# wesselb/gpar

Hardware: AMD Instinct MI355X
Metric: logpdf_per_s (higher is better)
Workload: dtype f64; 1 GPU; C3 dense GPAR log marginal likelihood: n=16384 m=4 p=8 markov=2 linear+nonlinear output kernels, noise=0.1, inputs resident in HBM

## Files before the change

### gpar_amd/csrc/gemm_f64.h

```cpp
#pragma once
#include "common.h"
#include <stdlib.h>

namespace gpar {

constexpr int GEMM_BM = 128;
constexpr int GEMM_BN = 128;
constexpr int GEMM_BK = 16;
constexpr int GEMM_LDKC = 18;
constexpr int GEMM_LDMC = 144;
constexpr int GEMM_TILE = 2304;
constexpr int GEMM_LDS_BYTES = 4 * GEMM_TILE * 8;
#ifndef GPAR_GEMM_EPI_PRIO
#define GPAR_GEMM_EPI_PRIO 3
#endif
#ifndef GPAR_GEMM_NT_STORE
#define GPAR_GEMM_NT_STORE 1
#endif
#ifndef GPAR_GEMM_PRELOAD_C
#define GPAR_GEMM_PRELOAD_C 1
#endif
constexpr int GEMM_LDT = 66;

struct GemmArgs {
    const double* A;
    const double* B;
    double* C;
    int m, n, k;
    int lda, ldb, ldc;
    double alpha, beta;
    int flags;
    int tiles_m, tiles_n;
    int fastA, fastB, fastC;
    int ksplit;
    long long part_stride;
    long long batch_a, batch_b, batch_c;
    int nfull, ntail;
    long long* stamps;
    long long* stage_stamps;
    const int* pred;
    int pred_sense;
};

typedef double gpar_d2 __attribute__((ext_vector_type(2)));
typedef double gpar_d4 __attribute__((ext_vector_type(4)));

template <bool KC, int FAST, int ROWS = 128>
__device__ __forceinline__ void gemm_gload(const double* __restrict__ g, int ld, int r0, int rmax, int k0,
                                           int kmax, bool lower, int t, gpar_d2 (&reg)[ROWS / 32]) {
    if (FAST) {
#pragma unroll
        for (int q = 0; q < ROWS / 32; ++q) {
            const int c = t + 256 * q;
            if (KC) {
                const int r = c >> 3, kk = (c & 7) * 2;
                const int row = (FAST == 2) ? min(r0 + r, rmax - 1) : r0 + r;
                reg[q] = *reinterpret_cast<const gpar_d2*>(g + (size_t)row * ld + k0 + kk);
            } else {
                const int kk = c / (ROWS / 2), r = (c % (ROWS / 2)) * 2;
                reg[q] = *reinterpret_cast<const gpar_d2*>(g + (size_t)(k0 + kk) * ld + r0 + r);
            }
        }
    } else {
#pragma unroll
        for (int q = 0; q < ROWS / 32; ++q) {
            const int c = t + 256 * q;
            int r, kk, r1, kk1;
            if (KC) { r = r0 + (c >> 3); kk = k0 + (c & 7) * 2; r1 = r; kk1 = kk + 1; }
            else { kk = k0 + c / (ROWS / 2); r = r0 + (c % (ROWS / 2)) * 2; r1 = r + 1; kk1 = kk; }
            const bool ok0 = r < rmax && kk < kmax && (!lower || kk <= r);
            const bool ok1 = r1 < rmax && kk1 < kmax && (!lower || kk1 <= r1);
            const int rc = min(r, rmax - 1), kc = min(kk, kmax - 1), rc1 = min(r1, rmax - 1), kc1 = min(kk1, kmax - 1);
            const double v0 = KC ? g[(size_t)rc * ld + kc] : g[(size_t)kc * ld + rc];
            const double v1 = KC ? g[(size_t)rc1 * ld + kc1] : g[(size_t)kc1 * ld + rc1];
            reg[q] = gpar_d2{ok0 ? v0 : 0.0, ok1 ? v1 : 0.0};
        }
    }
}

template <bool KC, int ROWS = 128>
__device__ __forceinline__ void gemm_sstore(double* __restrict__ s, int t, const gpar_d2 (&reg)[ROWS / 32]) {
#pragma unroll
    for (int q = 0; q < ROWS / 32; ++q) {
        const int c = t + 256 * q;
        if (KC) {
            const int r = c >> 3, kk = (c & 7) * 2;
            *reinterpret_cast<gpar_d2*>(s + r * GEMM_LDKC + kk) = reg[q];
        } else {
            const int kk = c / (ROWS / 2), r = (c % (ROWS / 2)) * 2;
            *reinterpret_cast<gpar_d2*>(s + kk * GEMM_LDMC + r) = reg[q];
        }
    }
}

template <bool A_KC, bool B_KC, int FAST, int BM>
__device__ __forceinline__ void gemm_mainloop(const GemmArgs& p, double* smem, gpar_d4 (&acc)[BM / 32][4], int m0, int n0,
                                              int kbeg, int kend, int nk, bool a_lower, int t, int lane, int wm, int wn) {
    gpar_d2 ra[BM / 32], rb[4];
    if (nk > 0) {
        gemm_gload<A_KC, FAST, BM>(p.A, p.lda, m0, p.m, kbeg, kend, a_lower, t, ra);
        gemm_gload<B_KC, FAST>(p.B, p.ldb, n0, p.n, kbeg, kend, false, t, rb);
        gemm_sstore<A_KC, BM>(smem, t, ra);
        gemm_sstore<B_KC>(smem + GEMM_TILE, t, rb);
    }
    __syncthreads();

    const int l15 = lane & 15, lk = lane >> 4;
    for (int kt = 0; kt < nk; ++kt) {
        const double* As = smem + (kt & 1) * 2 * GEMM_TILE;
        const double* Bs = As + GEMM_TILE;
        const bool more = kt + 1 < nk;
        __builtin_amdgcn_s_setprio(1);
#pragma unroll
        for (int k4 = 0; k4 < 4; ++k4) {
            const int kk = k4 * 4 + lk;
            double af[BM / 32], bf[4];
#pragma unroll
            for (int mi = 0; mi < BM / 32; ++mi) {
                const int r = wm * (BM / 2) + 16 * mi + l15;
                af[mi] = A_KC ? As[r * GEMM_LDKC + kk] : As[kk * GEMM_LDMC + r];
            }
#pragma unroll
            for (int nj = 0; nj < 4; ++nj) {
                const int c = wn * 64 + 16 * nj + l15;
                bf[nj] = B_KC ? Bs[c * GEMM_LDKC + kk] : Bs[kk * GEMM_LDMC + c];
            }
#pragma unroll
            for (int mi = 0; mi < BM / 32; ++mi)
#pragma unroll
                for (int nj = 0; nj < 4; ++nj)
                    acc[mi][nj] = __builtin_amdgcn_mfma_f64_16x16x4f64(af[mi], bf[nj], acc[mi][nj], 0, 0, 0);
            if (k4 == 0 && more) {
                gemm_gload<A_KC, FAST, BM>(p.A, p.lda, m0, p.m, kbeg + (kt + 1) * GEMM_BK, kend, a_lower, t, ra);
                gemm_gload<B_KC, FAST>(p.B, p.ldb, n0, p.n, kbeg + (kt + 1) * GEMM_BK, kend, false, t, rb);
            }
        }
        __builtin_amdgcn_s_setprio(0);
        if (more) {
            double* An = smem + ((kt + 1) & 1) * 2 * GEMM_TILE;
            gemm_sstore<A_KC, BM>(An, t, ra);
            gemm_sstore<B_KC>(An + GEMM_TILE, t, rb);
        }
        __syncthreads();
    }
}

template <bool A_KC, bool B_KC, int FAST, int BM>
__device__ __forceinline__ void gemm_stage(const GemmArgs& p, const double* __restrict__ As, const double* __restrict__ Bs,
                                           gpar_d4 (&acc)[BM / 32][4], int m0, int n0, int knext, int kend, int t, int l15, int lk,
                                           int wm, int wn, gpar_d2 (&ra)[BM / 32], gpar_d2 (&rb)[4]) {
    __builtin_amdgcn_s_setprio(1);
#pragma unroll
    for (int k4 = 0; k4 < 4; ++k4) {
        const int kk = k4 * 4 + lk;
        double af[BM / 32], bf[4];
#pragma unroll
        for (int mi = 0; mi < BM / 32; ++mi) {
            const int r = wm * (BM / 2) + 16 * mi + l15;
            af[mi] = A_KC ? As[r * GEMM_LDKC + kk] : As[kk * GEMM_LDMC + r];
        }
#pragma unroll
        for (int nj = 0; nj < 4; ++nj) {
            const int c = wn * 64 + 16 * nj + l15;
            bf[nj] = B_KC ? Bs[c * GEMM_LDKC + kk] : Bs[kk * GEMM_LDMC + c];
        }
#pragma unroll
        for (int mi = 0; mi < BM / 32; ++mi)
#pragma unroll
            for (int nj = 0; nj < 4; ++nj) {
                acc[mi][nj] = __builtin_amdgcn_mfma_f64_16x16x4f64(af[mi], bf[nj], acc[mi][nj], 0, 0, 0);
            }
        if (k4 == 0) {
            gemm_gload<A_KC, FAST, BM>(p.A, p.lda, m0, p.m, knext, kend, false, t, ra);
            gemm_gload<B_KC, FAST>(p.B, p.ldb, n0, p.n, knext, kend, false, t, rb);
        }
    }
    __builtin_amdgcn_s_setprio(0);
}

template <bool A_KC, bool B_KC, int FAST, int BM, bool PRELOAD = false>
__device__ __forceinline__ void gemm_mainloop_pf2(const GemmArgs& p, double* smem, gpar_d4 (&acc)[BM / 32][4], int m0, int n0,
                                                  int kbeg, int kend, int nk, int t, int lane, int wm, int wn) {
    static_assert(FAST != 0, "branch-free loads only");
    if (nk <= 0) return;
    gpar_d2 ra0[BM / 32], rb0[4], ra1[BM / 32], rb1[4];
    double* buf0 = smem;
    double* buf1 = smem + 2 * GEMM_TILE;
    const int klast = kbeg + (nk - 1) * GEMM_BK;
    gemm_gload<A_KC, FAST, BM>(p.A, p.lda, m0, p.m, kbeg, kend, false, t, ra0);
    gemm_gload<B_KC, FAST>(p.B, p.ldb, n0, p.n, kbeg, kend, false, t, rb0);
    gemm_gload<A_KC, FAST, BM>(p.A, p.lda, m0, p.m, min(kbeg + GEMM_BK, klast), kend, false, t, ra1);
    gemm_gload<B_KC, FAST>(p.B, p.ldb, n0, p.n, min(kbeg + GEMM_BK, klast), kend, false, t, rb1);
    if (PRELOAD) {
        const int wmu = __builtin_amdgcn_readfirstlane(wm), wnu = __builtin_amdgcn_readfirstlane(wn);
        const double* cw = p.C + (size_t)(m0 + wmu * (BM / 2)) * p.ldc + n0 + wnu * 64;
        const unsigned voff = ((unsigned)(lane >> 4) * (unsigned)p.ldc + (unsigned)(lane & 15)) * 8u;
        const double sgn = p.alpha;
#pragma unroll
        for (int mi = 0; mi < BM / 32; ++mi)
#pragma unroll
            for (int v = 0; v < 4; ++v) {
                const char* cr = reinterpret_cast<const char*>(cw + (size_t)(16 * mi + 4 * v) * p.ldc);
#pragma unroll
                for (int nj = 0; nj < 4; ++nj) acc[mi][nj][v] = sgn * *reinterpret_cast<const double*>(cr + voff + 128 * nj);
            }
    }
    gemm_sstore<A_KC, BM>(buf0, t, ra0);
    gemm_sstore<B_KC>(buf0 + GEMM_TILE, t, rb0);
    __syncthreads();
    const int l15 = lane & 15, lk = lane >> 4;
#ifdef GPAR_GEMM_STAGE_STAMPS
#define GEMM_STAGE_STAMP(stage, which)                                                                                     \
    do {                                                                                                                   \
        if (p.stage_stamps && t == 0 && blockIdx.x >= 1024 && blockIdx.x < 1088 && (stage) < 40)                           \
            p.stage_stamps[((size_t)(blockIdx.x - 1024) * 40 + (stage)) * 3 + (which)] =                                     \
                (GPAR_GEMM_STAGE_STAMPS == 2) ? (long long)__builtin_amdgcn_s_memtime() : (long long)__builtin_amdgcn_s_memrealtime(); \
    } while (0)
#else
#define GEMM_STAGE_STAMP(stage, which) do {} while (0)
#endif
    for (int kt = 0; kt < nk; kt += 2) {
        GEMM_STAGE_STAMP(kt, 0);
        gemm_stage<A_KC, B_KC, FAST, BM>(p, buf0, buf0 + GEMM_TILE, acc, m0, n0, min(kbeg + (kt + 2) * GEMM_BK, klast), kend, t, l15,
                                     lk, wm, wn, ra0, rb0);
        GEMM_STAGE_STAMP(kt, 1);
        if (kt + 1 >= nk) break;
        gemm_sstore<A_KC, BM>(buf1, t, ra1);
        gemm_sstore<B_KC>(buf1 + GEMM_TILE, t, rb1);
        GEMM_STAGE_STAMP(kt, 2);
        __syncthreads();
        GEMM_STAGE_STAMP(kt + 1, 0);
        gemm_stage<A_KC, B_KC, FAST, BM>(p, buf1, buf1 + GEMM_TILE, acc, m0, n0, min(kbeg + (kt + 3) * GEMM_BK, klast), kend, t, l15,
                                     lk, wm, wn, ra1, rb1);
        GEMM_STAGE_STAMP(kt + 1, 1);
        if (kt + 2 >= nk) break;
        gemm_sstore<A_KC, BM>(buf0, t, ra0);
        gemm_sstore<B_KC>(buf0 + GEMM_TILE, t, rb0);
        GEMM_STAGE_STAMP(kt + 1, 2);
        __syncthreads();
    }
    __syncthreads();
}

template <int MI, bool HAS_BETA>
__device__ __forceinline__ void gemm_epilogue_lds(const GemmArgs& p, double* smem, gpar_d4 (&acc)[MI][4], int row0, int col0,
                                                  double alpha, double beta, int w, int lane) {
    const int l15 = lane & 15, lk = lane >> 4;
    double* S = smem + w * GEMM_TILE;
    const int rrow = lane >> 5, rcol = (lane & 31) * 2;
    double* cbase = p.C + (size_t)(row0 + rrow) * p.ldc + col0 + rcol;
    gpar_d2 cv[2][8];
    if (HAS_BETA) {
#pragma unroll
        for (int q = 0; q < 8; ++q) cv[0][q] = *reinterpret_cast<const gpar_d2*>(cbase + (size_t)(2 * q) * p.ldc);
    }
#pragma unroll
    for (int h = 0; h < MI; ++h) {
#pragma unroll
        for (int nj = 0; nj < 4; ++nj)
#pragma unroll
            for (int v = 0; v < 4; ++v) S[(lk + 4 * v) * GEMM_LDT + 16 * nj + l15] = acc[h][nj][v];
        if (HAS_BETA && h < MI - 1) {
#pragma unroll
            for (int q = 0; q < 8; ++q)
                cv[(h + 1) & 1][q] = *reinterpret_cast<const gpar_d2*>(cbase + (size_t)(16 * (h + 1) + 2 * q) * p.ldc);
        }
        __builtin_amdgcn_fence(__ATOMIC_RELEASE, "wavefront");
        __builtin_amdgcn_wave_barrier();
        __builtin_amdgcn_fence(__ATOMIC_ACQUIRE, "wavefront");
        gpar_d2 v2[8];
#pragma unroll
        for (int q = 0; q < 8; ++q) v2[q] = *reinterpret_cast<const gpar_d2*>(S + (2 * q + rrow) * GEMM_LDT + rcol);
        __builtin_amdgcn_fence(__ATOMIC_RELEASE, "wavefront");
        __builtin_amdgcn_wave_barrier();
#pragma unroll
        for (int q = 0; q < 8; ++q) {
            gpar_d2 o = v2[q] * alpha;
            if (HAS_BETA) o = gpar_d2{fma(beta, cv[h & 1][q][0], o[0]), fma(beta, cv[h & 1][q][1], o[1])};
#if GPAR_GEMM_NT_STORE
            __builtin_nontemporal_store(o, reinterpret_cast<gpar_d2*>(cbase + (size_t)(16 * h + 2 * q) * p.ldc));
#else
            *reinterpret_cast<gpar_d2*>(cbase + (size_t)(16 * h + 2 * q) * p.ldc) = o;
#endif
        }
    }
}

template <bool TA, bool TB, int BM>
__device__ __forceinline__ void gemm_tile_body(GemmArgs& p, double* smem, const int blk, const int nblk, const int tile0) {
    constexpr int MI = BM / 32;
    constexpr bool A_KC = !TA;
    constexpr bool B_KC = TB;

    const long long t_start = p.stamps ? (long long)__builtin_amdgcn_s_memrealtime() : 0;
    p.A += (size_t)blockIdx.z * p.batch_a;
    p.B += (size_t)blockIdx.z * p.batch_b;
    p.C += (size_t)blockIdx.z * p.batch_c;
    int idx = 0, tm = -1, tn = -1;
    const bool tri_rect = !(p.flags & GPAR_GEMM_C_LOWER) && BM == GEMM_BM;
    if (tri_rect && (p.flags & GPAR_GEMM_K_TO_COL) && !(p.flags & (GPAR_GEMM_K_FROM_ROW | GPAR_GEMM_A_LOWER)) && (p.tiles_n & 7) == 0) {
        const int b = blk, xcd = b & 7, j = b >> 3;
        tn = p.tiles_n - 1 - ((j / p.tiles_m) * 8 + xcd);
        tm = j % p.tiles_m;
    } else if (p.flags & (GPAR_GEMM_K_FROM_ROW | GPAR_GEMM_A_LOWER | GPAR_GEMM_K_TO_COL)) {
        idx = tile0 + blk / (GEMM_BM / BM);
    } else {
        const int nb = nblk / (GEMM_BM / BM), b = blk / (GEMM_BM / BM);
        const int xcd = b & 7, q = nb >> 3, r = nb & 7;
        idx = tile0 + (xcd < r ? xcd * (q + 1) : r * (q + 1) + (xcd - r) * q) + (b >> 3);
    }
    if (tm >= 0) {
    } else if (p.flags & GPAR_GEMM_C_LOWER) {
        const int tri = p.tiles_n * (p.tiles_n + 1) / 2;
        if (idx < tri) {
            tm = (int)((sqrt(8.0 * (double)idx + 1.0) - 1.0) * 0.5);
            while ((tm + 1) * (tm + 2) / 2 <= idx) ++tm;
            while (tm * (tm + 1) / 2 > idx) --tm;
            tn = idx - tm * (tm + 1) / 2;
        } else {
            const int r = idx - tri;
            tm = p.tiles_n + r / p.tiles_n;
            tn = r % p.tiles_n;
        }
    } else {
        tm = idx / p.tiles_n;
        tn = idx % p.tiles_n;
    }
    const int m0 = tm * GEMM_BM + (BM == GEMM_BM ? 0 : (int)(blk & 1) * BM), n0 = tn * GEMM_BN;

    const int t = threadIdx.x, lane = t & 63, w = t >> 6;
    const int wm = w >> 1, wn = w & 1;
    const bool a_lower = (p.flags & GPAR_GEMM_A_LOWER) != 0;
    int kend = a_lower ? min(p.k, m0 + BM) : p.k;
    if (p.flags & GPAR_GEMM_K_TO_COL) kend = min(kend, n0 + GEMM_BN);
    int kbeg = (p.flags & GPAR_GEMM_K_FROM_ROW) ? min(m0, kend) : 0;
    if (p.ksplit > 0) {
        kbeg = max(kbeg, (int)blockIdx.y * p.ksplit);
        kend = min(kend, ((int)blockIdx.y + 1) * p.ksplit);
        if (kend < kbeg) kend = kbeg;
        p.C += (size_t)blockIdx.y * p.part_stride;
    }
    const int nk = (kend - kbeg + GEMM_BK - 1) / GEMM_BK;

    gpar_d4 acc[MI][4];
#pragma unroll
    for (int i = 0; i < MI; ++i)
#pragma unroll
        for (int j = 0; j < 4; ++j) acc[i][j] = gpar_d4{0.0, 0.0, 0.0, 0.0};

    const bool fastk = p.fastA && p.fastB && !a_lower && ((kend - kbeg) % GEMM_BK == 0);
    const bool inner = (m0 + BM <= p.m) && (n0 + GEMM_BN <= p.n);
    const bool c_lower = (p.flags & GPAR_GEMM_C_LOWER) != 0;
    const bool preload = GPAR_GEMM_PRELOAD_C && fastk && inner && nk > 0 && p.ksplit <= 0 && p.beta == 1.0 &&
                         (p.alpha == 1.0 || p.alpha == -1.0) && (!c_lower || n0 + GEMM_BN - 1 <= m0);
    if (preload) gemm_mainloop_pf2<A_KC, B_KC, 1, BM, true>(p, smem, acc, m0, n0, kbeg, kend, nk, t, lane, wm, wn);
    else if (fastk && inner) gemm_mainloop_pf2<A_KC, B_KC, 1, BM>(p, smem, acc, m0, n0, kbeg, kend, nk, t, lane, wm, wn);
    else if (fastk && A_KC && B_KC) gemm_mainloop_pf2<A_KC, B_KC, 2, BM>(p, smem, acc, m0, n0, kbeg, kend, nk, t, lane, wm, wn);
    else gemm_mainloop<A_KC, B_KC, 0, BM>(p, smem, acc, m0, n0, kbeg, kend, nk, a_lower, t, lane, wm, wn);
    const long long t_main = p.stamps ? (long long)__builtin_amdgcn_s_memrealtime() : 0;
#if GPAR_GEMM_EPI_PRIO
    __builtin_amdgcn_s_setprio(GPAR_GEMM_EPI_PRIO);
#endif
    const int l15 = lane & 15, lk = lane >> 4;

    const int colw = n0 + wn * 64 + l15;
    const int roww = m0 + wm * (BM / 2) + lk;
    const double alpha = p.alpha, beta = preload ? 0.0 : p.beta;
    const bool interior = (m0 + BM <= p.m) && (n0 + GEMM_BN <= p.n) && (!c_lower || n0 + GEMM_BN - 1 <= m0);
    if (interior && p.fastC) {
        if (beta != 0.0) gemm_epilogue_lds<MI, true>(p, smem, acc, m0 + wm * (BM / 2), n0 + wn * 64, alpha, beta, w, lane);
        else gemm_epilogue_lds<MI, false>(p, smem, acc, m0 + wm * (BM / 2), n0 + wn * 64, alpha, beta, w, lane);
    } else if (interior) {
#pragma unroll
        for (int mi = 0; mi < MI; ++mi) {
            double cv[4][4];
            if (beta != 0.0) {
#pragma unroll
                for (int nj = 0; nj < 4; ++nj)
#pragma unroll
                    for (int v = 0; v < 4; ++v)
                        cv[nj][v] = p.C[(size_t)(roww + 16 * mi + 4 * v) * p.ldc + colw + 16 * nj];
            }
#pragma unroll
            for (int nj = 0; nj < 4; ++nj)
#pragma unroll
                for (int v = 0; v < 4; ++v) {
                    double x = alpha * acc[mi][nj][v];
                    if (beta != 0.0) x = fma(beta, cv[nj][v], x);
                    p.C[(size_t)(roww + 16 * mi + 4 * v) * p.ldc + colw + 16 * nj] = x;
                }
        }
    } else {
#pragma unroll
        for (int mi = 0; mi < MI; ++mi) {
            const int blk0 = m0 + wm * (BM / 2) + 16 * mi;
            if (blk0 >= p.m || (c_lower && n0 + wn * 64 > blk0 + 15)) continue;
#pragma unroll
            for (int v = 0; v < 4; ++v) {
                const int row = roww + 16 * mi + 4 * v;
                const int rowc = min(row, p.m - 1);
                double cv[4] = {0.0, 0.0, 0.0, 0.0};
                if (beta != 0.0) {
#pragma unroll
                    for (int nj = 0; nj < 4; ++nj) cv[nj] = p.C[(size_t)rowc * p.ldc + min(colw + 16 * nj, p.n - 1)];
                }
#pragma unroll
                for (int nj = 0; nj < 4; ++nj) {
                    const int col = colw + 16 * nj;
                    const bool ok = row < p.m && col < p.n && (!c_lower || col <= row);
                    double x = alpha * acc[mi][nj][v];
                    if (beta != 0.0) x = fma(beta, cv[nj], x);
                    if (ok) p.C[(size_t)row * p.ldc + col] = x;
                }
            }
        }
    }
    if (p.stamps && threadIdx.x == 0) {
        asm volatile("s_waitcnt vmcnt(0)" ::: "memory");
        p.stamps[blockIdx.x * 4 + 0] = t_start;
        p.stamps[blockIdx.x * 4 + 1] = t_main;
        p.stamps[blockIdx.x * 4 + 2] = (long long)__builtin_amdgcn_s_memrealtime();
        p.stamps[blockIdx.x * 4 + 3] = (long long)(__builtin_amdgcn_s_getreg((16 - 1) << 11 | 4) | (__builtin_amdgcn_s_getreg((4 - 1) << 11 | 20) << 16));
    }
}


template <bool TA, bool TB, int ROLE, int BM = 128>
__global__ __launch_bounds__(256, 2) void gemm_f64_kernel(GemmArgs p) {
    extern __shared__ __attribute__((aligned(16))) double smem[];
    if (ROLE == 0 && gpar_pred_skip(p.pred, p.pred_sense)) return;
    if (ROLE == 1 && BM == GEMM_BM && p.ntail > 0 && (int)blockIdx.x >= p.nfull)
        gemm_tile_body<TA, TB, 64>(p, smem, (int)blockIdx.x - p.nfull, 2 * p.ntail, p.nfull);
    else
        gemm_tile_body<TA, TB, BM>(p, smem, (int)blockIdx.x, ROLE == 1 && BM == GEMM_BM && p.ntail > 0 ? p.nfull : (int)gridDim.x, 0);
}

inline int gemm_num_tiles(int tiles_m, int tiles_n, int flags) {
    if (flags & GPAR_GEMM_C_LOWER) {
        const int tn = tiles_n < tiles_m ? tiles_n : tiles_m;
        return tn * (tn + 1) / 2 + (tiles_m - tn) * tn;
    }
    return tiles_m * tiles_n;
}

static int gemm_launch(int ta, int tb, int m, int n, int k, double alpha, const double* A, int lda,
                       const double* B, int ldb, double beta, double* C, int ldc, int flags, hipStream_t stream,
                       int role = 0, int batch = 1, long long batch_a = 0, long long batch_b = 0, long long batch_c = 0) {
    if (m <= 0 || n <= 0 || batch <= 0) return 0;
    GemmArgs p;
    p.batch_a = batch_a; p.batch_b = batch_b; p.batch_c = batch_c;
    p.A = A; p.B = B; p.C = C;
    p.m = m; p.n = n; p.k = k;
    p.lda = lda; p.ldb = ldb; p.ldc = ldc;
    p.alpha = alpha; p.beta = beta;
    p.flags = flags;
    p.tiles_m = gpar_ceil_div(m, GEMM_BM);
    p.tiles_n = gpar_ceil_div(n, GEMM_BN);
    if (flags & GPAR_GEMM_C_LOWER) {
        if (p.tiles_n > p.tiles_m) p.tiles_n = p.tiles_m;
    }
    p.fastA = gpar_aligned16(A) && (lda % 2 == 0);
    p.fastB = gpar_aligned16(B) && (ldb % 2 == 0);
    p.fastC = gpar_aligned16(C) && (ldc % 2 == 0);
    p.stamps = nullptr; p.stage_stamps = nullptr;
    p.pred = role == 0 ? g_pred.flag : nullptr; p.pred_sense = g_pred.sense;
    p.ksplit = 0;
    p.part_stride = 0;
    const int ntiles = gemm_num_tiles(p.tiles_m, p.tiles_n, flags);
    for (const void* fn : {reinterpret_cast<const void*>(&gemm_f64_kernel<false, false, 0>), reinterpret_cast<const void*>(&gemm_f64_kernel<false, true, 0>),
                           reinterpret_cast<const void*>(&gemm_f64_kernel<true, false, 0>), reinterpret_cast<const void*>(&gemm_f64_kernel<true, true, 0>),
                           reinterpret_cast<const void*>(&gemm_f64_kernel<false, true, 1>), reinterpret_cast<const void*>(&gemm_f64_kernel<false, true, 0, 64>),
                           reinterpret_cast<const void*>(&gemm_f64_kernel<false, true, 1, 64>), reinterpret_cast<const void*>(&gemm_f64_kernel<false, false, 0, 64>)})
        GPAR_HIP_TRY(gpar_set_max_lds(fn, 160 * 1024));
    static int half_tiles = -1;
    if (half_tiles < 0) { const char* e = getenv("GPAR_GEMM_HALF_TILES"); half_tiles = e ? atoi(e) : 256; }
    static int half_flags = -1;
    if (half_flags < 0) { const char* e = getenv("GPAR_GEMM_HALF_TILES_TRIANGULAR"); half_flags = e ? atoi(e) : 1; }
    const bool half = !ta && ntiles * batch <= half_tiles && k >= 64 &&
                      (half_flags || !(flags & (GPAR_GEMM_A_LOWER | GPAR_GEMM_K_FROM_ROW | GPAR_GEMM_K_TO_COL)));
    const int GEMM_LDS_REQ = GEMM_LDS_BYTES;
    p.nfull = ntiles; p.ntail = 0;
    static int mixed_tail = -1;
    if (mixed_tail < 0) { const char* e = getenv("GPAR_GEMM_MIXED_TAIL"); mixed_tail = e ? atoi(e) : 1; }
    if (mixed_tail && !half && role == 1 && !ta && tb && batch == 1 && k >= 64 && ntiles > 512 && ntiles % 512 != 0 && ntiles % 512 <= 256 &&
        !(flags & (GPAR_GEMM_A_LOWER | GPAR_GEMM_K_FROM_ROW | GPAR_GEMM_K_TO_COL))) {
        p.ntail = ntiles % 512;
        p.nfull = ntiles - p.ntail;
    }
    dim3 grid(half ? 2 * ntiles : p.nfull + 2 * p.ntail, 1, batch), block(256);
    if (half && role == 1) hipLaunchKernelGGL((gemm_f64_kernel<false, true, 1, 64>), grid, block, GEMM_LDS_REQ, stream, p);
    else if (half && tb) hipLaunchKernelGGL((gemm_f64_kernel<false, true, 0, 64>), grid, block, GEMM_LDS_REQ, stream, p);
    else if (half) hipLaunchKernelGGL((gemm_f64_kernel<false, false, 0, 64>), grid, block, GEMM_LDS_REQ, stream, p);
    else if (role == 1 && !ta && tb) hipLaunchKernelGGL((gemm_f64_kernel<false, true, 1>), grid, block, GEMM_LDS_REQ, stream, p);
    else if (!ta && !tb) hipLaunchKernelGGL((gemm_f64_kernel<false, false, 0>), grid, block, GEMM_LDS_REQ, stream, p);
    else if (!ta && tb) hipLaunchKernelGGL((gemm_f64_kernel<false, true, 0>), grid, block, GEMM_LDS_REQ, stream, p);
    else if (ta && !tb) hipLaunchKernelGGL((gemm_f64_kernel<true, false, 0>), grid, block, GEMM_LDS_REQ, stream, p);
    else hipLaunchKernelGGL((gemm_f64_kernel<true, true, 0>), grid, block, GEMM_LDS_REQ, stream, p);
    GPAR_LAUNCH_CHECK();
    return 0;
}

__global__ __launch_bounds__(256) void gemm_splitk_reduce_kernel(const double* __restrict__ ws, long long part_stride, int splits,
                                                                 int m, int n, double alpha, double beta, double* __restrict__ C,
                                                                 int ldc, int lower) {
    const int col = blockIdx.x * blockDim.x + threadIdx.x;
    const int row = blockIdx.y;
    if (col >= n || row >= m || (lower && col > row)) return;
    double s = 0.0;
    for (int q = 0; q < splits; ++q) s += ws[(size_t)q * part_stride + (size_t)row * n + col];
    double* dst = C + (size_t)row * ldc + col;
    *dst = (beta != 0.0) ? fma(beta, *dst, alpha * s) : alpha * s;
}

static int gemm_splitk_launch(int ta, int tb, int m, int n, int k, double alpha, const double* A, int lda, const double* B,
                              int ldb, double beta, double* C, int ldc, int flags, int splits, double* workspace,
                              hipStream_t stream) {
    if (m <= 0 || n <= 0) return 0;
    if (splits <= 1 || !workspace) return gemm_launch(ta, tb, m, n, k, alpha, A, lda, B, ldb, beta, C, ldc, flags, stream);
    GemmArgs p;
    p.batch_a = p.batch_b = p.batch_c = 0;
    p.A = A; p.B = B; p.C = workspace;
    p.m = m; p.n = n; p.k = k;
    p.lda = lda; p.ldb = ldb; p.ldc = n;
    p.alpha = 1.0; p.beta = 0.0;
    p.flags = flags;
    p.tiles_m = gpar_ceil_div(m, GEMM_BM);
    p.tiles_n = gpar_ceil_div(n, GEMM_BN);
    if ((flags & GPAR_GEMM_C_LOWER) && p.tiles_n > p.tiles_m) p.tiles_n = p.tiles_m;
    p.fastA = gpar_aligned16(A) && (lda % 2 == 0);
    p.fastB = gpar_aligned16(B) && (ldb % 2 == 0);
    p.fastC = gpar_aligned16(workspace) && (n % 2 == 0) && (((long long)m * n) % 2 == 0);
    p.stamps = nullptr; p.stage_stamps = nullptr;
    p.pred = nullptr; p.pred_sense = 0;
    const int len = gpar_ceil_div(gpar_ceil_div(k, splits), GEMM_BK) * GEMM_BK;
    p.ksplit = len;
    p.nfull = 0; p.ntail = 0;
    p.part_stride = (long long)m * n;
    const int nsl = gpar_ceil_div(k, len);
    const int ntiles = gemm_num_tiles(p.tiles_m, p.tiles_n, flags);
    for (const void* fn : {reinterpret_cast<const void*>(&gemm_f64_kernel<false, false, 0>), reinterpret_cast<const void*>(&gemm_f64_kernel<false, true, 0>),
                           reinterpret_cast<const void*>(&gemm_f64_kernel<true, false, 0>), reinterpret_cast<const void*>(&gemm_f64_kernel<true, true, 0>)})
        GPAR_HIP_TRY(gpar_set_max_lds(fn, 160 * 1024));
    dim3 grid(ntiles, nsl), block(256);
    if (!ta && !tb) hipLaunchKernelGGL((gemm_f64_kernel<false, false, 0>), grid, block, GEMM_LDS_BYTES, stream, p);
    else if (!ta && tb) hipLaunchKernelGGL((gemm_f64_kernel<false, true, 0>), grid, block, GEMM_LDS_BYTES, stream, p);
    else if (ta && !tb) hipLaunchKernelGGL((gemm_f64_kernel<true, false, 0>), grid, block, GEMM_LDS_BYTES, stream, p);
    else hipLaunchKernelGGL((gemm_f64_kernel<true, true, 0>), grid, block, GEMM_LDS_BYTES, stream, p);
    hipLaunchKernelGGL(gemm_splitk_reduce_kernel, dim3(gpar_ceil_div(n, 256), m), dim3(256), 0, stream, (const double*)workspace,
                       p.part_stride, nsl, m, n, alpha, beta, C, ldc, (flags & GPAR_GEMM_C_LOWER) ? 1 : 0);
    GPAR_LAUNCH_CHECK();
    return 0;
}

}
```

Measured before the change: 5.585 logpdf/s.

## Precompute global load addresses, prefetch LDS fragments ahead, split LDS stores into MFMA loop

Global-load addresses for the A/B tiles are now computed once per block as a uniform base pointer plus per-lane offsets, instead of being rebuilt in every stage. LDS fragments for the next k4 step are double-buffered in registers so their reads overlap the current MFMAs. The shared-memory stores for the next tile are moved inside the MFMA loop at k4 == 2 and 3 rather than issued after the stage. The aim is to cut VALU address work and hide LDS latency, at the cost of more registers and a restructured loop tail. The fast path is also restricted to leading dimensions small enough for 32-bit offsets.

```diff
diff --git a/gpar_amd/csrc/gemm_f64.h b/gpar_amd/csrc/gemm_f64.h
--- a/gpar_amd/csrc/gemm_f64.h
+++ b/gpar_amd/csrc/gemm_f64.h
@@ -145,34 +145,121 @@
     }
 }
 
+#ifndef GPAR_GEMM_ADDR_ONCE
+#define GPAR_GEMM_ADDR_ONCE 1
+#endif
+#ifndef GPAR_GEMM_FRAG_AHEAD
+#define GPAR_GEMM_FRAG_AHEAD 1
+#endif
+#ifndef GPAR_GEMM_SPLIT_STORE
+#define GPAR_GEMM_SPLIT_STORE 1
+#endif
+constexpr int GEMM_FAST_LD_MAX = 1 << 21;
+
+template <bool KC, int FAST, int ROWS>
+struct GemmSrc {
+    const char* base;
+    size_t kstep;
+    unsigned qstep;
+    unsigned voff[FAST == 2 ? ROWS / 32 : 1];
+};
+
+template <bool KC, int FAST, int ROWS>
+__device__ __forceinline__ GemmSrc<KC, FAST, ROWS> gemm_src(const double* __restrict__ g, int ld, int r0, int rmax, int t) {
+    static_assert(FAST != 0, "branch-free loads only");
+    GemmSrc<KC, FAST, ROWS> s;
+    r0 = __builtin_amdgcn_readfirstlane(r0);
+    if (FAST == 2) r0 = min(r0, rmax - 1);
+    if (KC) {
+        const int r = t >> 3, kk = (t & 7) * 2;
+        s.base = reinterpret_cast<const char*>(g + (size_t)r0 * ld);
+        s.kstep = 8;
+        s.qstep = 32u * (unsigned)ld * 8u;
+        if (FAST == 2) {
+#pragma unroll
+            for (int q = 0; q < ROWS / 32; ++q) s.voff[q] = ((unsigned)(min(r0 + r + 32 * q, rmax - 1) - r0) * (unsigned)ld + (unsigned)kk) * 8u;
+        } else {
+            s.voff[0] = ((unsigned)r * (unsigned)ld + (unsigned)kk) * 8u;
+        }
+    } else {
+        const int kk = t / (ROWS / 2), r = (t % (ROWS / 2)) * 2;
+        s.base = reinterpret_cast<const char*>(g + r0);
+        s.kstep = (size_t)ld * 8;
+        s.qstep = (unsigned)(512 / ROWS) * (unsigned)ld * 8u;
+        s.voff[0] = ((unsigned)kk * (unsigned)ld + (unsigned)r) * 8u;
+        if (FAST == 2) {
+#pragma unroll
+            for (int q = 1; q < ROWS / 32; ++q) s.voff[q] = s.voff[0] + q * s.qstep;
+        }
+    }
+    return s;
+}
+
+typedef const __attribute__((address_space(1))) char* gpar_gptr;
+typedef const __attribute__((address_space(1))) gpar_d2* gpar_gptr_d2;
+__device__ __forceinline__ gpar_gptr gemm_uniform(const char* ptr) {
+    const unsigned long long a = reinterpret_cast<unsigned long long>(ptr);
+    const unsigned lo = __builtin_amdgcn_readfirstlane((unsigned)a), hi = __builtin_amdgcn_readfirstlane((unsigned)(a >> 32));
+    return (gpar_gptr)(((unsigned long long)hi << 32) | lo);
+}
+
+template <bool KC, int FAST, int ROWS>
+__device__ __forceinline__ void gemm_gload_src(const GemmSrc<KC, FAST, ROWS>& s, int k0, gpar_d2 (&reg)[ROWS / 32]) {
+    const char* sb = s.base + (size_t)k0 * s.kstep;
+#pragma unroll
+    for (int q = 0; q < ROWS / 32; ++q) {
+        unsigned vo = s.voff[FAST == 2 ? q : 0];
+        asm volatile("" : "+v"(vo));
+        reg[q] = *(gpar_gptr_d2)(gemm_uniform(sb + (FAST == 2 ? (size_t)0 : (size_t)q * s.qstep)) + vo);
+    }
+}
+
+template <bool A_KC, bool B_KC, int BM>
+__device__ __forceinline__ void gemm_frag(const double* __restrict__ As, const double* __restrict__ Bs, int k4, int l15, int lk,
+                                          int wm, int wn, double (&af)[BM / 32], double (&bf)[4]) {
+    const int kk = k4 * 4 + lk;
+#pragma unroll
+    for (int mi = 0; mi < BM / 32; ++mi) {
+        const int r = wm * (BM / 2) + 16 * mi + l15;
+        af[mi] = A_KC ? As[r * GEMM_LDKC + kk] : As[kk * GEMM_LDMC + r];
+    }
+#pragma unroll
+    for (int nj = 0; nj < 4; ++nj) {
+        const int c = wn * 64 + 16 * nj + l15;
+        bf[nj] = B_KC ? Bs[c * GEMM_LDKC + kk] : Bs[kk * GEMM_LDMC + c];
+    }
+}
+
 template <bool A_KC, bool B_KC, int FAST, int BM>
 __device__ __forceinline__ void gemm_stage(const GemmArgs& p, const double* __restrict__ As, const double* __restrict__ Bs,
-                                           gpar_d4 (&acc)[BM / 32][4], int m0, int n0, int knext, int kend, int t, int l15, int lk,
-                                           int wm, int wn, gpar_d2 (&ra)[BM / 32], gpar_d2 (&rb)[4]) {
+                                           gpar_d4 (&acc)[BM / 32][4], const GemmSrc<A_KC, FAST, BM>& srcA,
+                                           const GemmSrc<B_KC, FAST, 128>& srcB, int m0, int n0, int knext, int kend, int t, int l15, int lk,
+                                           int wm, int wn, double (&af)[2][BM / 32], double (&bf)[2][4], gpar_d2 (&ra)[BM / 32],
+                                           gpar_d2 (&rb)[4], double* __restrict__ An, double* __restrict__ Bn, const gpar_d2 (&sa)[BM / 32],
+                                           const gpar_d2 (&sb)[4]) {
     __builtin_amdgcn_s_setprio(1);
 #pragma unroll
     for (int k4 = 0; k4 < 4; ++k4) {
-        const int kk = k4 * 4 + lk;
-        double af[BM / 32], bf[4];
+        const int cur = GPAR_GEMM_FRAG_AHEAD ? (k4 & 1) : 0;
+        if (!GPAR_GEMM_FRAG_AHEAD) gemm_frag<A_KC, B_KC, BM>(As, Bs, k4, l15, lk, wm, wn, af[0], bf[0]);
+        else if (k4 < 3) gemm_frag<A_KC, B_KC, BM>(As, Bs, k4 + 1, l15, lk, wm, wn, af[cur ^ 1], bf[cur ^ 1]);
 #pragma unroll
         for (int mi = 0; mi < BM / 32; ++mi) {
-            const int r = wm * (BM / 2) + 16 * mi + l15;
-            af[mi] = A_KC ? As[r * GEMM_LDKC + kk] : As[kk * GEMM_LDMC + r];
-        }
-#pragma unroll
-        for (int nj = 0; nj < 4; ++nj) {
-            const int c = wn * 64 + 16 * nj + l15;
-            bf[nj] = B_KC ? Bs[c * GEMM_LDKC + kk] : Bs[kk * GEMM_LDMC + c];
-        }
-#pragma unroll
-        for (int mi = 0; mi < BM / 32; ++mi)
 #pragma unroll
             for (int nj = 0; nj < 4; ++nj) {
-                acc[mi][nj] = __builtin_amdgcn_mfma_f64_16x16x4f64(af[mi], bf[nj], acc[mi][nj], 0, 0, 0);
-            }
+                acc[mi][nj] = __builtin_amdgcn_mfma_f64_16x16x4f64(af[cur][mi], bf[cur][nj], acc[mi][nj], 0, 0, 0);
+            }
+            if (GPAR_GEMM_SPLIT_STORE && mi == 0 && k4 == 2) gemm_sstore<A_KC, BM>(An, t, sa);
+            if (GPAR_GEMM_SPLIT_STORE && mi == 0 && k4 == 3) gemm_sstore<B_KC>(Bn, t, sb);
+        }
         if (k4 == 0) {
+#if GPAR_GEMM_ADDR_ONCE
+            gemm_gload_src<A_KC, FAST, BM>(srcA, knext, ra);
+            gemm_gload_src<B_KC, FAST, 128>(srcB, knext, rb);
+#else
             gemm_gload<A_KC, FAST, BM>(p.A, p.lda, m0, p.m, knext, kend, false, t, ra);
             gemm_gload<B_KC, FAST>(p.B, p.ldb, n0, p.n, knext, kend, false, t, rb);
+#endif
         }
     }
     __builtin_amdgcn_s_setprio(0);
@@ -187,10 +274,19 @@
     double* buf0 = smem;
     double* buf1 = smem + 2 * GEMM_TILE;
     const int klast = kbeg + (nk - 1) * GEMM_BK;
+    const GemmSrc<A_KC, FAST, BM> srcA = gemm_src<A_KC, FAST, BM>(p.A, p.lda, m0, p.m, t);
+    const GemmSrc<B_KC, FAST, 128> srcB = gemm_src<B_KC, FAST, 128>(p.B, p.ldb, n0, p.n, t);
+#if GPAR_GEMM_ADDR_ONCE
+    gemm_gload_src<A_KC, FAST, BM>(srcA, kbeg, ra0);
+    gemm_gload_src<B_KC, FAST, 128>(srcB, kbeg, rb0);
+    gemm_gload_src<A_KC, FAST, BM>(srcA, min(kbeg + GEMM_BK, klast), ra1);
+    gemm_gload_src<B_KC, FAST, 128>(srcB, min(kbeg + GEMM_BK, klast), rb1);
+#else
     gemm_gload<A_KC, FAST, BM>(p.A, p.lda, m0, p.m, kbeg, kend, false, t, ra0);
     gemm_gload<B_KC, FAST>(p.B, p.ldb, n0, p.n, kbeg, kend, false, t, rb0);
     gemm_gload<A_KC, FAST, BM>(p.A, p.lda, m0, p.m, min(kbeg + GEMM_BK, klast), kend, false, t, ra1);
     gemm_gload<B_KC, FAST>(p.B, p.ldb, n0, p.n, min(kbeg + GEMM_BK, klast), kend, false, t, rb1);
+#endif
     if (PRELOAD) {
         const int wmu = __builtin_amdgcn_readfirstlane(wm), wnu = __builtin_amdgcn_readfirstlane(wn);
         const double* cw = p.C + (size_t)(m0 + wmu * (BM / 2)) * p.ldc + n0 + wnu * 64;
@@ -209,6 +305,8 @@
     gemm_sstore<B_KC>(buf0 + GEMM_TILE, t, rb0);
     __syncthreads();
     const int l15 = lane & 15, lk = lane >> 4;
+    double af[2][BM / 32], bf[2][4];
+    if (GPAR_GEMM_FRAG_AHEAD) gemm_frag<A_KC, B_KC, BM>(buf0, buf0 + GEMM_TILE, 0, l15, lk, wm, wn, af[0], bf[0]);
 #ifdef GPAR_GEMM_STAGE_STAMPS
 #define GEMM_STAGE_STAMP(stage, which)                                                                                     \
     do {                                                                                                                   \
@@ -219,27 +317,38 @@
 #else
 #define GEMM_STAGE_STAMP(stage, which) do {} while (0)
 #endif
-    for (int kt = 0; kt < nk; kt += 2) {
+    int kt = 0;
+    for (; kt + 2 <= nk; kt += 2) {
         GEMM_STAGE_STAMP(kt, 0);
-        gemm_stage<A_KC, B_KC, FAST, BM>(p, buf0, buf0 + GEMM_TILE, acc, m0, n0, min(kbeg + (kt + 2) * GEMM_BK, klast), kend, t, l15,
-                                     lk, wm, wn, ra0, rb0);
+        gemm_stage<A_KC, B_KC, FAST, BM>(p, buf0, buf0 + GEMM_TILE, acc, srcA, srcB, m0, n0, min(kbeg + (kt + 2) * GEMM_BK, klast), kend,
+                                         t, l15, lk, wm, wn, af, bf, ra0, rb0, buf1, buf1 + GEMM_TILE, ra1, rb1);
         GEMM_STAGE_STAMP(kt, 1);
-        if (kt + 1 >= nk) break;
-        gemm_sstore<A_KC, BM>(buf1, t, ra1);
-        gemm_sstore<B_KC>(buf1 + GEMM_TILE, t, rb1);
+        if (!GPAR_GEMM_SPLIT_STORE) {
+            gemm_sstore<A_KC, BM>(buf1, t, ra1);
+            gemm_sstore<B_KC>(buf1 + GEMM_TILE, t, rb1);
+        }
         GEMM_STAGE_STAMP(kt, 2);
         __syncthreads();
+        if (GPAR_GEMM_FRAG_AHEAD) gemm_frag<A_KC, B_KC, BM>(buf1, buf1 + GEMM_TILE, 0, l15, lk, wm, wn, af[0], bf[0]);
         GEMM_STAGE_STAMP(kt + 1, 0);
-        gemm_stage<A_KC, B_KC, FAST, BM>(p, buf1, buf1 + GEMM_TILE, acc, m0, n0, min(kbeg + (kt + 3) * GEMM_BK, klast), kend, t, l15,
-                                     lk, wm, wn, ra1, rb1);
+        gemm_stage<A_KC, B_KC, FAST, BM>(p, buf1, buf1 + GEMM_TILE, acc, srcA, srcB, m0, n0, min(kbeg + (kt + 3) * GEMM_BK, klast), kend,
+                                         t, l15, lk, wm, wn, af, bf, ra1, rb1, buf0, buf0 + GEMM_TILE, ra0, rb0);
         GEMM_STAGE_STAMP(kt + 1, 1);
-        if (kt + 2 >= nk) break;
-        gemm_sstore<A_KC, BM>(buf0, t, ra0);
-        gemm_sstore<B_KC>(buf0 + GEMM_TILE, t, rb0);
+        if (!GPAR_GEMM_SPLIT_STORE) {
+            gemm_sstore<A_KC, BM>(buf0, t, ra0);
+            gemm_sstore<B_KC>(buf0 + GEMM_TILE, t, rb0);
+        }
         GEMM_STAGE_STAMP(kt + 1, 2);
         __syncthreads();
-    }
-    __syncthreads();
+        if (GPAR_GEMM_FRAG_AHEAD) gemm_frag<A_KC, B_KC, BM>(buf0, buf0 + GEMM_TILE, 0, l15, lk, wm, wn, af[0], bf[0]);
+    }
+    if (kt < nk) {
+        GEMM_STAGE_STAMP(kt, 0);
+        gemm_stage<A_KC, B_KC, FAST, BM>(p, buf0, buf0 + GEMM_TILE, acc, srcA, srcB, m0, n0, klast, kend, t, l15, lk, wm, wn, af, bf, ra0,
+                                         rb0, buf1, buf1 + GEMM_TILE, ra1, rb1);
+        GEMM_STAGE_STAMP(kt, 1);
+        __syncthreads();
+    }
 }
 
 template <int MI, bool HAS_BETA>
@@ -348,7 +457,7 @@
 #pragma unroll
         for (int j = 0; j < 4; ++j) acc[i][j] = gpar_d4{0.0, 0.0, 0.0, 0.0};
 
-    const bool fastk = p.fastA && p.fastB && !a_lower && ((kend - kbeg) % GEMM_BK == 0);
+    const bool fastk = p.fastA && p.fastB && !a_lower && ((kend - kbeg) % GEMM_BK == 0) && p.lda <= GEMM_FAST_LD_MAX && p.ldb <= GEMM_FAST_LD_MAX;
     const bool inner = (m0 + BM <= p.m) && (n0 + GEMM_BN <= p.n);
     const bool c_lower = (p.flags & GPAR_GEMM_C_LOWER) != 0;
     const bool preload = GPAR_GEMM_PRELOAD_C && fastk && inner && nk > 0 && p.ksplit <= 0 && p.beta == 1.0 &&
```

After: 5.660 logpdf/s, median of 6. +1.3%, better.
